# pyprob/pyprob

Measured on AMD Instinct MI355X. Metric: ic_train_traces_per_sec, higher is better.
Workload: dtype f32; 1 GPU; GaussianUnknownMean IC training, offline traces resident in HBM, LSTM hidden=512, batch=1024 per GPU; traces_in_hbm=1000000, params=1643583, global_batch=1024, parallelism=dp1, optimizer=Adam lr=1e-3*sqrt(world), launch=one Python iteration per step (ICEngine.train_step), eager launches, prewarm_steps=5670, minibatches_resident=976, minibatch_walk=step i trains minibatch (i * 1) mod 976 of the resident dataset

## Files before the change

### include/pyprob_amd.h

```cpp
#ifndef PYPROB_AMD_H
#define PYPROB_AMD_H

#include <stddef.h>
#include <stdint.h>

#ifdef __cplusplus
extern "C" {
#endif

#define PP_ABI_VERSION 15
#define PP_MAX_OBS 8
#define PP_MAX_LSTM_DEPTH 4
#define PP_MAX_OBS_DEPTH 4

#define PP_EINVAL   (-1)
#define PP_ENOSPACE (-2)
#define PP_ENODEV   (-3)
#define PP_EHIP     (-4)

#define PP_HEAD_NORMAL_MIXTURE       0
#define PP_HEAD_TRUNCNORMAL_MIXTURE  1
#define PP_HEAD_CATEGORICAL          2
#define PP_HEAD_BERNOULLI            4
#define PP_HEAD_POISSON_TN_MIXTURE   3

int         pp_abi_version(void);
const char* pp_last_error(void);
int         pp_device_count(void);

typedef struct pp_addr {
    int32_t kind;
    int32_t n_out;
    int32_t hid;
    int32_t smp_in;
    int32_t dtype_id;
    int32_t _pad;
    int64_t addr_emb;
    int64_t dtype_emb;
    int64_t smp_w;
    int64_t smp_b;
    int64_t w1, b1;
    int64_t w2, b2;
} pp_addr;

typedef struct pp_net {
    int32_t n_obs;
    int32_t obs_in[PP_MAX_OBS];
    int32_t obs_hid[PP_MAX_OBS];
    int32_t obs_out[PP_MAX_OBS];
    int64_t obs_w0[PP_MAX_OBS], obs_b0[PP_MAX_OBS], obs_w1[PP_MAX_OBS], obs_b1[PP_MAX_OBS];
    int32_t e_obs;
    int32_t smp_dim, addr_dim, dtype_dim;
    int64_t fin_w0, fin_b0, fin_w1, fin_b1;
    int32_t lstm_in;
    int32_t lstm_dim;
    int64_t w_ih, w_hh, b_ih, b_hh;
    int32_t n_addr;
    int32_t n_dtype;
    const pp_addr* addrs;
    const int64_t* addr_table;
    int64_t n_params;
    int32_t lstm_depth;
    int32_t _pad2;
    int64_t lstm_w_ih[PP_MAX_LSTM_DEPTH], lstm_w_hh[PP_MAX_LSTM_DEPTH], lstm_b_ih[PP_MAX_LSTM_DEPTH], lstm_b_hh[PP_MAX_LSTM_DEPTH];
    int32_t obs_depth[PP_MAX_OBS];
    int64_t obs_w[PP_MAX_OBS][PP_MAX_OBS_DEPTH], obs_b[PP_MAX_OBS][PP_MAX_OBS_DEPTH];
    int32_t obs_kind[PP_MAX_OBS];
    int32_t obs_shape[PP_MAX_OBS][3];
    int32_t obs_feat[PP_MAX_OBS];
    int32_t _pad3;
    int64_t obs_conv_w[PP_MAX_OBS][5], obs_conv_b[PP_MAX_OBS][5];
} pp_net;

#define PP_OBS_FEEDFORWARD 0
#define PP_OBS_CNN2D5C     1
#define PP_PROF_CNN_FWD 32
#define PP_PROF_CNN_BWD 48

size_t pp_cnn2d5c_workspace_bytes(const pp_net* net, int32_t o, int32_t n_images);
int pp_cnn2d5c_forward(const pp_net* net, int32_t o, const float* params, const float* x, int32_t n_images,
                       float* features_out, void* workspace, size_t workspace_bytes, void* stream);
int pp_cnn2d5c_backward(const pp_net* net, int32_t o, const float* params, const float* d_features, int32_t n_images,
                        float* grads, void* workspace, size_t workspace_bytes, int32_t flags, void* stream);

#define PP_ADDR_TABLE_COLS 8
#define PP_AT_KIND 0
#define PP_AT_SMP_IN 1
#define PP_AT_ADDR_EMB 2
#define PP_AT_DTYPE_EMB 3
#define PP_AT_SMP_W 4
#define PP_AT_SMP_B 5
#define PP_AT_N_OUT 6
#define PP_AT_RESERVED 7

typedef struct pp_batch {
    int32_t n_traces;
    int32_t n_rows;
    int32_t t_max;
    int32_t obs_width;
    const int32_t* n_active;
    const int32_t* row_off;
    const int32_t* grp_off;
    const float*   obs;
    const float*   value;
    const float*   prior;
    const int32_t* addr;
    const int32_t* prev_row;
    const int32_t* grp_rows;
    const int32_t* trace;
    const int32_t* row_off_dev;
    const int32_t* nxt_off;
    const int32_t* nxt_rows;
} pp_batch;

typedef struct pp_pack_info {
    int64_t n_traces, n_rows, t_max, device_words;
    int64_t obs, value, prior, addr, prev_row, grp_rows, trace, row_off_dev, nxt_rows;
    int64_t n_active, row_off, grp_off, nxt_off;
    int64_t order;
    int64_t src_row;
} pp_pack_info;

int64_t pp_pack_words(int32_t n_traces, int64_t n_rows, int32_t t_max, int32_t obs_width, int32_t n_addr);

int pp_pack_ragged(const int32_t* trace_len, const int32_t* addr_ids, const float* values, const float* prior,
                   int32_t prior_width, const float* obs, int32_t n_traces, int32_t obs_width, int32_t n_addr,
                   void* out, int64_t out_words, pp_pack_info* info);

typedef struct pp_shard_columns {
    const int32_t* trace_len;
    const int64_t* row_off;
    const float*   obs;
    const float*   value;
    const float*   prior;
    const int32_t* addr;
    const int32_t* addr_remap;
} pp_shard_columns;

int pp_pack_indexed(const pp_shard_columns* shards, int32_t n_shards, const int64_t* first, const int64_t* ids,
                    int32_t n_ids, int32_t obs_width, int32_t n_addr, void* out, int64_t out_words, pp_pack_info* info);


size_t pp_ic_workspace_bytes(const pp_net* net, int32_t n_traces, int32_t n_rows);

#define PP_LOSS_BACKWARD   1
#define PP_LOSS_ZERO_GRADS 2
#define PP_LOSS_KEEP_LP    4

int pp_ic_loss(const pp_net* net, const pp_batch* batch, const float* params , float* grads ,
               void* workspace , size_t workspace_bytes, float* loss_out ,
               int32_t* status_out , float* lp_out , int32_t flags, void* stream);

#define PP_ADAM_ZERO_GRADS 1
#define PP_ADAM_SCRATCH 1056
#define PP_ADAM_SEEN 1027
int pp_adam_step(float* params, float* grads, float* exp_avg, float* exp_avg_sq, int64_t n_params,
                 const int32_t* chunk_tensor, const float* active, int32_t* tensor_step, int32_t* scratch,
                 int32_t n_tensors, float lr, float beta1, float beta2, float eps, float weight_decay, float grad_scale,
                 int32_t flags, const int32_t* skip, void* stream);

int pp_sgd_step(float* params, float* grads, float* momentum_buf, int64_t n_params, const int32_t* chunk_tensor,
                const float* active, int32_t n_tensors, float lr, float momentum, int32_t nesterov, float weight_decay,
                float grad_scale, int32_t flags, const int32_t* skip, void* stream);

#define PP_LARC_SCRATCH_FLOATS(n_params, n_tensors) (2 * ((n_params) / 1024) + (n_tensors))
int pp_larc_scale(const float* params, float* grads, int64_t n_params, const int32_t* chunk_tensor, const float* active,
                  int32_t n_tensors, float lr, float weight_decay, float grad_scale, float trust_coefficient, float eps,
                  float epsilon, int32_t clip, float* scratch, const int32_t* skip, void* stream);

typedef struct pp_train_buffers {
    float* params; float* grads; float* exp_avg; float* exp_avg_sq;
    const int32_t* chunk_tensor; int32_t* tensor_step; int32_t* adam_scratch;
    void* workspace; size_t workspace_bytes;
    void* staging; void* device_batch; int64_t slot_words;
    float* loss_ring; int32_t* status_ring;
    int32_t n_tensors; int32_t n_slots;
    int32_t dp_world; int32_t dp_n_skip;
    int64_t dp_skip_off[4], dp_skip_cnt[4];
} pp_train_buffers;

typedef struct pp_tensor_roles {
    const int32_t* off;
    const int32_t* addr;
    const int32_t* role;
} pp_tensor_roles;

int64_t pp_train_slot_words(int32_t n_traces, int64_t n_rows, int32_t t_max, int32_t obs_width, int32_t n_addr,
                            int32_t n_tensors);

int pp_train_sync(void);
int pp_train_resident(const pp_net* net, const pp_train_buffers* tb, const pp_batch* const* batches,
                      const float* const* active, int32_t n_steps, const float* lr, float beta1, float beta2, float eps,
                      float weight_decay, int32_t grads_clean, void* stream);

int pp_train_steps(const pp_net* net, const pp_train_buffers* buffers, const pp_tensor_roles* roles,
                   const pp_shard_columns* shards, int32_t n_shards, const int64_t* first, int32_t obs_width,
                   const int64_t* ids, const int64_t* step_off, int32_t n_steps, const float* lr ,
                   float beta1, float beta2, float eps, float weight_decay, int32_t grads_clean,
                   int64_t* addr_iterations, void* stream);


size_t pp_is_workspace_bytes(const pp_net* net, int32_t n);

int pp_is_init(const pp_net* net, const float* params, const float* obs, float* e_out, void* workspace,
               size_t workspace_bytes, void* stream);

int pp_is_step(const pp_net* net, const float* params, int32_t addr_id, int32_t prev_addr_id, int32_t n,
               const float* e_obs_vec, const float* prev_value, const float* prior, int32_t prior_stride,
               float* h, float* c, int32_t state_rows, const float* value_in, float* value_out, float* logq_out,
               uint64_t seed, uint64_t offset, void* workspace, size_t workspace_bytes, void* stream);

int pp_is_step_rows(const pp_net* net, const float* params, int32_t addr_id, int32_t prev_addr_id, int32_t n,
                    const float* e_obs_vec, const float* prev_value, const float* prior, int32_t prior_stride,
                    float* h, float* c, int32_t state_rows, const int64_t* rows, const float* value_in, float* value_out,
                    float* logq_out, uint64_t seed, uint64_t offset, void* workspace, size_t workspace_bytes, void* stream);
int pp_is_step_fused_supported(const pp_net* net, int32_t addr_id, int32_t n);
int pp_is_statement_rows(const pp_net* net, const float* params, int32_t addr_id, int32_t prev_addr_id, int32_t n,
                         const float* e_obs_vec, const float* prev_value_full, const float* prior, int32_t prior_stride,
                         float* h, float* c, int32_t state_rows, const int64_t* rows, float* value_full, float* lw_full,
                         int32_t prior_kind, uint64_t seed, uint64_t offset, void* workspace, size_t workspace_bytes,
                         void* stream);

int pp_logweight_accumulate(int32_t kind, const float* p0, int32_t p0_stride, const float* p1, int32_t p1_stride,
                            const float* x, int32_t x_stride, float scale, float* lw , float* lp_out,
                            int32_t n, void* stream);

int pp_logweight_accumulate_rows(int32_t kind, const float* p0, int32_t p0_stride, const float* p1, int32_t p1_stride,
                                 const float* x, int32_t x_stride, float scale, float* lw ,
                                 const int64_t* rows, int32_t m, void* stream);

int pp_copy_rows(const float* src, int32_t src_stride, float* dst , const int64_t* rows, int32_t m, void* stream);

#define PP_PARTITION_SCRATCH(m) (((m) + 1023) / 1024 + 1)
int pp_partition_rows(const uint8_t* cond, const int64_t* rows, int32_t m, int64_t* rows_true, int64_t* rows_false,
                      int32_t* counts, int32_t* scratch, void* stream);
int pp_partition_rows_polled(const uint8_t* cond, const int64_t* rows, int32_t m, int64_t* rows_true, int64_t* rows_false,
                             int32_t* counts , int32_t seq, int32_t* scratch, void* stream);

typedef struct pp_lw_term {
    int32_t kind, p0_stride, p1_stride, x_stride;
    const float *p0, *p1, *x;
    float scale;
} pp_lw_term;
int pp_logweight_terms(const pp_lw_term* terms, int32_t count, float* lw , int32_t n, int32_t overwrite,
                       void* stream);

int pp_is_step_net(const pp_net* net, const float* params, int32_t addr_id, int32_t prev_addr_id, int32_t n,
                   const float* e_obs_vec, const float* prev_value, float* h, float* c, int32_t state_rows, void* workspace,
                   size_t workspace_bytes, void* stream);
int pp_is_first_statement_supported(const pp_net* net, int32_t addr_id);
int pp_is_first_statement(const pp_net* net, const float* params, const float* obs, int32_t addr_id, float* e_out, float* h, float* c,
                          void* workspace, size_t workspace_bytes, void* stream);
int pp_is_fused(const pp_net* net, int32_t addr_id, int32_t n, const float* prior , const pp_lw_term* terms,
                const int32_t* term_flags, int32_t n_terms, float* value , float* lw , int32_t overwrite,
                uint64_t seed, uint64_t offset, double* stats_out , double* stats_scratch, void* workspace,
                size_t workspace_bytes, void* stream);

#define PP_IS_GROUP_STATS_BYTES(m) ((size_t)((m) > 256 ? (m) : 256) * 48)
#define PP_GROUPS_PRIOR_PER_PARTICLE 2
size_t pp_is_batch_workspace_bytes(const pp_net* net, int32_t n_groups);
int pp_is_batch_first(const pp_net* net, const float* params, const float* obs , int32_t addr_id, int32_t n_groups,
                      float* y_out , int64_t ldy, float* h_out, float* c_out , void* workspace,
                      size_t workspace_bytes, void* stream);
int pp_is_fused_groups(const pp_net* net, int32_t addr_id, int32_t n_groups, int32_t n_per, const float* y , int64_t ldy,
                       const float* prior , const pp_lw_term* terms, const int32_t* term_flags, int32_t n_terms,
                       float* value , float* lw , int32_t overwrite, uint64_t seed, uint64_t offset,
                       double* stats_out , void* workspace, size_t workspace_bytes, void* stream);

int pp_is_batch_bias(const pp_net* net, const float* params, int32_t addr_id, int32_t prev_addr_id, int32_t n_groups,
                     int32_t ws_groups, int32_t first_group, const float* h_prev ,
                     float* bias_out , void* workspace, size_t workspace_bytes, void* stream);
int pp_is_statement_groups(const pp_net* net, const float* params, int32_t addr_id, int32_t prev_addr_id, int32_t n_groups,
                           int32_t n_per, const float* bias , const float* c0 ,
                           const float* prev_value , const float* prior, int32_t prior_stride, float* h, float* c,
                           float* value , float* lw , int32_t prior_kind, uint64_t seed, uint64_t offset,
                           float* y_out , int64_t ldy, void* workspace, size_t workspace_bytes,
                           void* stream);

int pp_prior_draw(int32_t kind, const float* p0, int32_t p0_stride, const float* p1, int32_t p1_stride, int32_t n, uint64_t seed,
                  uint64_t offset, uint32_t stream_id, float* out , void* stream);

int pp_obs_draw(int32_t kind, const float* p0, int64_t p0_row_stride, int32_t p0_elem_stride, const float* p1, int64_t p1_row_stride,
                int32_t p1_elem_stride, int32_t n, int32_t k, uint64_t seed, uint64_t offset, uint32_t stream_id,
                float* out , void* stream);

int pp_axpy(float scale, const float* term, float* lw, int32_t n, void* stream);

#define PP_IS_STATS_SCRATCH 6144
int pp_is_stats(const float* lw, const float* x, int32_t n, double* out, double* scratch, void* stream);

#define PP_DIST_MAX_KIND 13
#define PP_DIST_MAX_TERMS 8
#define PP_DIST_MAX_ROUNDS 64
typedef struct pp_dist {
    int32_t kind;
    int32_t p_stride[4];
    const float* p[4];
} pp_dist;
typedef struct pp_dist_term {
    pp_dist d;
    const float* x; int32_t x_stride;
    float scale;
} pp_dist_term;

int pp_dist_logweight(const pp_dist_term* terms, int32_t count, float* lw , float* lp_out, const int64_t* rows,
                      int32_t m, int32_t n, void* stream);

int pp_dist_draw(const pp_dist* d, const int64_t* rows, int32_t m, int32_t n, uint64_t seed, uint64_t offset, uint32_t stream_id,
                 float* out , void* stream);

#define PP_MIX_MAX_COMPONENTS 16
typedef struct pp_mixture {
    int32_t count;
    int32_t probs_stride;
    const float* probs;
    pp_dist comp[PP_MIX_MAX_COMPONENTS];
} pp_mixture;

int pp_mix_logweight(const pp_mixture* mix, const float* x, int32_t x_stride, float scale, float* lw , float* lp_out,
                     const int64_t* rows, int32_t m, int32_t n, void* stream);

int pp_mix_draw(const pp_mixture* mix, const int64_t* rows, int32_t m, int32_t n, uint64_t seed, uint64_t offset,
                uint32_t stream_id, float* out , void* stream);

typedef struct pp_obs_operand { const float* p; int64_t row_stride; int32_t elem_stride; int32_t _pad; } pp_obs_operand;
int pp_obs_logweight(int32_t kind, const pp_obs_operand params[4], pp_obs_operand x, int32_t k, float scale, float* lw ,
                     float* lp_out, const int64_t* rows, int32_t m, int32_t n, void* stream);

typedef struct pp_gemm_args {
    const float* A; int64_t lda; const int32_t* a_idx;
    const float* B; int64_t ldb; const int32_t* b_idx;
    float*       C; int64_t ldc; const int32_t* c_idx;
    int32_t M, N, K;
    int32_t a_kmajor, b_kmajor;
    const float* bias;
    const float* bias2;
    const float* mask; int64_t ldmask;
    int32_t relu;
    int32_t accumulate;
    float*       colsum;
    int32_t split_k;
    int32_t _pad;
} pp_gemm_args;

int pp_gemm_f32(const pp_gemm_args* args, void* stream);
int pp_gemm_f32_grouped(const pp_gemm_args* args, int32_t count, void* stream);

int pp_colsum_f32(const float* X, int64_t ldx, const int32_t* row_idx, int32_t n_rows, int32_t n_cols,
                  float* out, float* out2, void* stream);

int pp_lstm_input_gather(const pp_net* net, const float* params, const float* E, const int32_t* trace_of_row,
                         const float* value, const int32_t* addr, const int32_t* prev_row, int32_t n_rows,
                         float* X, int64_t ldx, void* stream);

int pp_lstm_cell_fwd(float* G, const float* c_prev, float* c, float* h, int32_t n, int32_t H, void* stream);
int pp_lstm_cell_bwd(float* G, const float* c_prev, const float* c, const float* dh, float* dc_carry,
                     int32_t n, int32_t n_next, int32_t H, void* stream);

int pp_head_logprob(int32_t kind, const float* y, int64_t ldy, const int32_t* rows, const float* value,
                    const float* prior, int32_t n, int32_t n_out, float grad_scale, float* lp_out, float* dy,
                    float* loss_acc, int32_t* nonfinite, void* stream);

int pp_debug_wgrad_plan(const pp_gemm_args* products, const int32_t* zero_blocks, int32_t count, int64_t* out, int32_t cap,
                        int32_t* n_blocks);
int pp_prof_arm(int32_t which, int32_t max_samples);
int pp_prof_stride(int32_t stride);
int pp_prof_collect(float* ms_out, int32_t cap, int32_t* n_out, double* flops_out);

int pp_dp_unique_id(const char* rccl_path, void* id_out );
int pp_dp_init(const char* rccl_path, const void* unique_id , int32_t rank, int32_t world);
int pp_dp_world(void);
int pp_dp_destroy(void);
int pp_dp_allreduce(float* base , const int64_t* off , const int64_t* cnt , int32_t n, void* stream);
int pp_dp_reduce_grads(float* grads_full, int64_t n_params, int32_t n_tensors, const float* presence, const int32_t* status,
                       const int64_t* skip_off , const int64_t* skip_cnt , int32_t n_skip, float* loss_out,
                       int32_t* status_out, void* stream);

int pp_dp_overlap(const int64_t* off , const int64_t* cnt , int32_t n);
int pp_dp_overlap_stats(int32_t arm, float* us_out);

int pp_debug_timeline(long long* buf );
int pp_debug_wgtrace(long long* buf, int32_t cap, int32_t mode);
int pp_debug_clock_probe(int32_t iters, long long* out , float* sink , void* stream);

#ifdef __cplusplus
}
#endif
#endif
```

### pyprob_amd/csrc/wgrad_t1.hip

```cpp
#include "wgrad_t1.hpp"

#include <stdlib.h>

#include <algorithm>

namespace pp {

extern long long* g_wgtrace;
extern int g_wgtrace_cap, g_wgtrace_mode;

namespace {

typedef float f32x16 __attribute__((ext_vector_type(16)));

constexpr int WG_RING = 8;

struct Pair {
    float a0, a1, b0, b1;
};

template <bool GATHER>
__device__ __forceinline__ void wgrad_kloop(f32x16 (&acc)[2][2], const float* __restrict__ A, const float* __restrict__ B,
                                            const int32_t* __restrict__ bidx, const int lda, const int ldb, const int M, const int N,
                                            const int m0, const int n0, const int kb, const int ke, const int lane,
                                            const bool hm, const bool hn) {
    const int l31 = lane & 31, h = lane >> 5;
    const float* pa0 = A + min(m0 + l31, M - 1);
    const float* pa1 = A + min(m0 + 32 + l31, M - 1);
    const float* pb0 = B + min(n0 + l31, N - 1);
    const float* pb1 = B + min(n0 + 32 + l31, N - 1);
    int idxA = 0, idxB = 0;
    if (GATHER) idxA = bidx[min(kb + lane, ke - 1)];
    auto load = [&](int pidx, Pair& p) {
        const int k = kb + 2 * pidx + h;
        const int kc = min(k, ke - 1);
        const float keep = k < ke ? 1.0f : 0.0f;
        p.a0 = pa0[(int64_t)kc * lda] * keep;
        p.a1 = pa1[(int64_t)kc * lda] * keep;
        int kb2 = kc;
        if (GATHER) {
            if ((pidx & 31) == 0) {
                const int nb = (pidx >> 5) + 1;
                const int v = bidx[min(kb + 64 * nb + lane, ke - 1)];
                idxB = (nb & 1) ? v : idxB;
                idxA = (nb & 1) ? idxA : v;
            }
            const int v = ((pidx >> 5) & 1) ? idxB : idxA;
            const int sel = 2 * (pidx & 31);
            const int r0 = __builtin_amdgcn_readlane(v, sel), r1 = __builtin_amdgcn_readlane(v, sel + 1);
            kb2 = h ? r1 : r0;
        }
        p.b0 = pb0[(int64_t)kb2 * ldb];
        p.b1 = pb1[(int64_t)kb2 * ldb];
    };
    auto mma = [&](const Pair& p) {
        acc[0][0] = __builtin_amdgcn_mfma_f32_32x32x2f32(p.a0, p.b0, acc[0][0], 0, 0, 0);
        if (hn) acc[0][1] = __builtin_amdgcn_mfma_f32_32x32x2f32(p.a0, p.b1, acc[0][1], 0, 0, 0);
        if (hm) acc[1][0] = __builtin_amdgcn_mfma_f32_32x32x2f32(p.a1, p.b0, acc[1][0], 0, 0, 0);
        if (hm && hn) acc[1][1] = __builtin_amdgcn_mfma_f32_32x32x2f32(p.a1, p.b1, acc[1][1], 0, 0, 0);
    };
    Pair f[WG_RING];
    const int nfr = (ke - kb + 1) >> 1;
#pragma unroll
    for (int i = 0; i < WG_RING - 1; ++i) load(i, f[i]);
    int i0 = 0;
    for (; i0 + WG_RING <= nfr; i0 += WG_RING) {
#pragma unroll
        for (int j = 0; j < WG_RING; ++j) {
            load(i0 + j + WG_RING - 1, f[(j + WG_RING - 1) % WG_RING]);
            mma(f[j]);
        }
    }
    const int nrem = nfr - i0;
#pragma unroll
    for (int j = 0; j < WG_RING - 1; ++j)
        if (j < nrem) mma(f[j]);
}

__global__ __launch_bounds__(512, 4) void wgrad_t1_kernel(const WgradT1Args g, const AuxJobs aux) {
    __shared__ float lds[8192];
    const long long t_start = g.trace ? wall_clock64() : 0;
    const int aux_lo = g.aux_first ? 0 : g.n_blocks;
    const int bx = (int)blockIdx.x - (g.aux_first ? aux.n_blocks : 0);
    if ((int)blockIdx.x >= aux_lo && (int)blockIdx.x < aux_lo + aux.n_blocks) {
        int jb = (int)blockIdx.x - aux_lo + g.aux_rot;
        if (jb >= aux.n_blocks) jb -= aux.n_blocks;
        aux_job_run(aux, jb, lds);
        if (g.trace && threadIdx.x == 0) {
            long long* tr = g.trace + 8 * blockIdx.x;
            tr[0] = t_start; tr[1] = wall_clock64(); tr[2] = 100; tr[3] = 0;
        }
        return;
    }
    int pi = 0;
#pragma unroll
    for (int q = 1; q < WGRAD_T1_MAX; ++q)
        if (q < g.n_prob && bx >= g.p[q].first) pi = q;
    const float* const A = g.p[pi].A;
    const float* const B = g.p[pi].B;
    float* const C = g.p[pi].C;
    const int32_t* const bidx = g.p[pi].bidx;
    const int lda = g.p[pi].lda, ldb = g.p[pi].ldb, ldc = g.p[pi].ldc, M = g.p[pi].M, N = g.p[pi].N, nt = g.p[pi].nt;
    const int K = g.p[pi].K, ks = g.p[pi].ks;
    const int local = bx - g.p[pi].first;
    const int mtg = g.p[pi].mtg;
    int s, tm, tn;
    if (mtg > 0) {
        const int r = local & 7, u = local >> 3;
        const int tmg = u % mtg, v = u / mtg;
        tn = v % nt;
        s = v / nt;
        tm = tmg * 8 + r;
        if (tm * 64 >= M) return;
    } else {
        const int tiles = ((M + 63) >> 6) * nt;
        s = local / tiles;
        const int t = local - s * tiles;
        tm = t / nt;
        tn = t - tm * nt;
    }
    const int tid = threadIdx.x, lane = tid & 63, l31 = lane & 31, h = lane >> 5;
    const int wave = __builtin_amdgcn_readfirstlane(tid >> 6);
    const int m0 = tm * 64, n0 = tn * 64;
    const int k0 = s * ks, k1 = min(K, k0 + ks);
    const int per = ((k1 - k0 + 15) >> 4) * 2;
    const int kb = k0 + wave * per, ke = min(k1, kb + per);
    f32x16 acc[2][2];
#pragma unroll
    for (int i = 0; i < 2; ++i)
#pragma unroll
        for (int j = 0; j < 2; ++j)
#pragma unroll
            for (int r = 0; r < 16; ++r) acc[i][j][r] = 0.0f;
    const bool hm = m0 + 32 < M, hn = n0 + 32 < N;
    if (kb < ke) {
        if (bidx) wgrad_kloop<true>(acc, A, B, bidx, lda, ldb, M, N, m0, n0, kb, ke, lane, hm, hn);
        else wgrad_kloop<false>(acc, A, B, bidx, lda, ldb, M, N, m0, n0, kb, ke, lane, hm, hn);
    }
    if (g.trace && threadIdx.x == 0) g.trace[8 * blockIdx.x + 4] = wall_clock64();
    float out[2][2][2];
#pragma unroll
    for (int qi = 0; qi < 2; ++qi) {
#pragma unroll
        for (int qj = 0; qj < 2; ++qj) {
            out[qi][qj][0] = out[qi][qj][1] = 0.0f;
            if ((qi && !hm) || (qj && !hn)) continue;
            if (qi + qj > 0) __syncthreads();
            float* mine = lds + wave * 1024 + lane;
#pragma unroll
            for (int r = 0; r < 16; ++r) mine[r * 64] = acc[qi][qj][r];
            __syncthreads();
#pragma unroll
            for (int e = 0; e < 2; ++e) {
                const int r = 2 * wave + e;
                float v = 0.0f;
#pragma unroll
                for (int w = 0; w < 8; ++w) v += lds[w * 1024 + r * 64 + lane];
                out[qi][qj][e] = v;
                if (!g.aux_first) {
                    const int gm = m0 + 32 * qi + (r & 3) + 8 * (r >> 2) + 4 * h;
                    const int gn = n0 + 32 * qj + l31;
                    if (gm < M && gn < N) atomicAdd(C + (int64_t)gm * ldc + gn, v);
                }
            }
        }
    }
#pragma unroll
    for (int qi = 0; qi < 2; ++qi)
#pragma unroll
        for (int qj = 0; qj < 2; ++qj) {
            if (!g.aux_first || (qi && !hm) || (qj && !hn)) continue;
#pragma unroll
            for (int e = 0; e < 2; ++e) {
                const int r = 2 * wave + e;
                const int gm = m0 + 32 * qi + (r & 3) + 8 * (r >> 2) + 4 * h;
                const int gn = n0 + 32 * qj + l31;
                if (gm < M && gn < N) atomicAdd(C + (int64_t)gm * ldc + gn, out[qi][qj][e]);
            }
        }
    if (g.trace && threadIdx.x == 0) {
        long long* tr = g.trace + 8 * blockIdx.x;
        tr[0] = t_start; tr[1] = wall_clock64(); tr[2] = pi; tr[3] = s;
    }
}

}

bool wgrad_t1_build(const pp_gemm_args* q, const GemmHole* holes, int n, WgradT1Args& out) {
    static const int env = getenv("PP_WGRAD_T1") ? atoi(getenv("PP_WGRAD_T1")) : 1;
    static const int env_s = 0;
    static const int env_xmap = getenv("PP_WGRAD_XMAP") ? atoi(getenv("PP_WGRAD_XMAP")) : 1;
    static const bool env_wgs_set = false;
    static const int env_wgs = 240;
    if (!env || deterministic_mode() || n <= 0) return false;
    out = WgradT1Args{};
    int np = 0;
    auto add = [&](const pp_gemm_args& a, int m_lo, int m_hi, int n_lo, int n_hi, int k_lo) -> bool {
        if (m_hi <= m_lo || n_hi <= n_lo || k_lo >= a.K) return true;
        if (np >= WGRAD_T1_MAX) return false;
        WgradT1Prob& p = out.p[np++];
        p.A = a.A + (int64_t)k_lo * a.lda + m_lo;
        p.bidx = a.b_idx ? a.b_idx + k_lo : nullptr;
        p.B = a.B + (a.b_idx ? 0 : (int64_t)k_lo * a.ldb) + n_lo;
        p.C = a.C + (int64_t)m_lo * a.ldc + n_lo;
        p.lda = (int)a.lda; p.ldb = (int)a.ldb; p.ldc = (int)a.ldc;
        p.M = m_hi - m_lo; p.N = n_hi - n_lo; p.nt = cdiv(p.N, 64);
        p.K = a.K - k_lo;
        return true;
    };
    for (int i = 0; i < n; ++i) {
        const pp_gemm_args& a = q[i];
        if (!a.a_kmajor || !a.b_kmajor || a.a_idx || a.c_idx || a.bias || a.bias2 || a.mask || a.relu || a.colsum ||
            !a.accumulate || a.K <= 0 || a.M <= 0 || a.N <= 0 || a.lda >= (1 << 30) || a.ldb >= (1 << 30) || a.ldc >= (1 << 30))
            return false;
        int mc[6] = {0, (int)a.M, 0, 0, 0, 0}, nc[6] = {0, (int)a.N, 0, 0, 0, 0};
        int nm = 2, nn = 2;
        GemmBlock z[2];
        int nz = 0;
        if (holes) {
            for (int b = 0; b < 2; ++b) {
                GemmBlock h = holes[i].b[b];
                h.m0 = std::max(h.m0, 0); h.n0 = std::max(h.n0, 0);
                h.m1 = std::min(h.m1, (int)a.M); h.n1 = std::min(h.n1, (int)a.N); h.k1 = std::min(h.k1, (int)a.K);
                if (h.m1 <= h.m0 || h.n1 <= h.n0 || h.k1 <= h.k0 || h.k0 > 0) continue;
                z[nz++] = h;
                mc[nm++] = h.m0; mc[nm++] = h.m1;
                nc[nn++] = h.n0; nc[nn++] = h.n1;
            }
        }
        std::sort(mc, mc + nm);
        std::sort(nc, nc + nn);
        nm = (int)(std::unique(mc, mc + nm) - mc);
        nn = (int)(std::unique(nc, nc + nn) - nc);
        for (int jn = 0; jn + 1 < nn; ++jn) {
            int run_lo = -1, run_hi = -1, run_k = 0;
            for (int jm = 0; jm + 1 < nm; ++jm) {
                int k_lo = 0;
                for (int b = 0; b < nz; ++b)
                    if (z[b].m0 <= mc[jm] && z[b].m1 >= mc[jm + 1] && z[b].n0 <= nc[jn] && z[b].n1 >= nc[jn + 1])
                        k_lo = std::max(k_lo, z[b].k1);
                if (run_lo >= 0 && k_lo == run_k) {
                    run_hi = mc[jm + 1];
                } else {
                    if (run_lo >= 0 && !add(a, run_lo, run_hi, nc[jn], nc[jn + 1], run_k)) return false;
                    run_lo = mc[jm]; run_hi = mc[jm + 1]; run_k = k_lo;
                }
            }
            if (run_lo >= 0 && !add(a, run_lo, run_hi, nc[jn], nc[jn + 1], run_k)) return false;
        }
    }
    if (np == 0) return false;
    int64_t tile_rows = 0;
    for (int i = 0; i < np; ++i) tile_rows += (int64_t)cdiv(out.p[i].M, 64) * out.p[i].nt * out.p[i].K;
    const int64_t blocks = env_wgs_set ? env_wgs : std::min<int64_t>(1536, std::max<int64_t>(env_wgs, tile_rows / 600));
    const int target_rows = (int)std::max<int64_t>(64, cdiv(tile_rows, std::max<int64_t>(blocks, 1)));
    out.n_prob = np;
    std::stable_sort(out.p, out.p + np, [](const WgradT1Prob& x, const WgradT1Prob& y) { return x.K > y.K; });
    int first = 0;
    for (int i = 0; i < np; ++i) {
        WgradT1Prob& p = out.p[i];
        int S = env_s > 0 ? env_s : (p.K + target_rows / 2) / target_rows;
        S = std::max(1, std::min(S, std::min(16, std::max(1, p.K / 64))));
        p.S = S;
        p.ks = ((cdiv(p.K, S) + 3) / 4) * 4;
        p.first = first;
        const int mt = cdiv(p.M, 64);
        p.mtg = (env_xmap && mt >= 8) ? cdiv(mt, 8) : 0;
        first += (p.mtg ? p.mtg * 8 : mt) * p.nt * S;
    }
    out.n_blocks = first;
    return true;
}

int wgrad_t1(const WgradT1Args& a, const AuxJobs* aux, hipStream_t st) {
    static const AuxJobs none{};
    const AuxJobs& j = aux ? *aux : none;
    const int blocks = a.n_blocks + (aux ? j.n_blocks : 0);
    WgradT1Args t = a;
    t.aux_first = (aux && a.n_blocks > 512) ? 1 : 0;
    const char* const env_rot = getenv("PP_WGRAD_JOBROT");
    if (aux && blocks <= 512 && !(env_rot && atoi(env_rot) == 0)) t.aux_rot = j.cs_first[j.n_colsum];
    if (g_wgtrace && g_wgtrace_mode == 1 && blocks <= g_wgtrace_cap) t.trace = g_wgtrace;
    hipLaunchKernelGGL(wgrad_t1_kernel, dim3(blocks), dim3(512), 0, st, t, j);
    PP_LAUNCH_CHECK("wgrad_t1");
    return 0;
}

}

extern "C" int pp_debug_wgrad_plan(const pp_gemm_args* q, const int32_t* zero_blocks, int32_t count, int64_t* out, int32_t cap,
                                   int32_t* n_blocks) {
    std::vector<pp::GemmHole> holes((size_t)std::max(count, 0));
    for (int i = 0; i < count && zero_blocks; ++i)
        for (int b = 0; b < 2; ++b) {
            const int32_t* z = zero_blocks + ((int64_t)i * 2 + b) * 6;
            holes[i].b[b] = pp::GemmBlock{z[0], z[1], z[2], z[3], z[4], z[5]};
        }
    pp::WgradT1Args a;
    if (!pp::wgrad_t1_build(q, zero_blocks ? holes.data() : nullptr, count, a)) return 0;
    if (n_blocks) *n_blocks = a.n_blocks;
    for (int i = 0; i < a.n_prob && i < cap; ++i) {
        const pp::WgradT1Prob& p = a.p[i];
        int src = -1;
        for (int k = 0; k < count; ++k)
            if (p.C >= q[k].C && p.C < q[k].C + (int64_t)q[k].M * q[k].ldc) src = k;
        int64_t* o = out + (int64_t)i * 10;
        o[0] = p.M; o[1] = p.N; o[2] = p.K; o[3] = p.S; o[4] = p.ks; o[5] = p.bidx ? 1 : 0; o[6] = p.first;
        o[7] = src >= 0 ? p.C - q[src].C : -1;
        o[8] = src >= 0 ? p.A - q[src].A : -1;
        o[9] = src >= 0 ? (p.bidx ? p.bidx - q[src].b_idx : (p.B - q[src].B)) : -1;
    }
    return a.n_prob;
}
```

### pyprob_amd/csrc/wgrad_t1.hpp

```cpp
#pragma once
#include "aux_jobs.hpp"
#include "common.hpp"

namespace pp {

constexpr int WGRAD_T1_MAX = 40;

struct WgradT1Prob {
    const float* A; const float* B; float* C;
    const int32_t* bidx;
    int lda, ldb, ldc;
    int M, N;
    int nt;
    int K, S, ks;
    int first;
    int mtg;
};

struct WgradT1Args {
    WgradT1Prob p[WGRAD_T1_MAX];
    int n_prob, n_blocks;
    int aux_first;
    int aux_rot;
    long long* trace;
};

bool wgrad_t1_build(const pp_gemm_args* q, const GemmHole* holes, int n, WgradT1Args& out);
int wgrad_t1(const WgradT1Args& a, const AuxJobs* aux, hipStream_t st);

}
```

### pyprob_amd/lib.py

```python
import ctypes as C
import os

HERE = os.path.dirname(os.path.abspath(__file__))
LIB_PATH = os.path.join(HERE, 'libpyprob_amd.so')

PP_ABI_VERSION = 15
PP_MAX_OBS = 8
PP_MAX_LSTM_DEPTH = 4
PP_MAX_OBS_DEPTH = 4
PP_MAX_MIXTURE_COMPONENTS = 16
PP_ADDR_TABLE_COLS = 8
PP_HEAD_NORMAL_MIXTURE, PP_HEAD_TRUNCNORMAL_MIXTURE, PP_HEAD_CATEGORICAL, PP_HEAD_POISSON_TN_MIXTURE = 0, 1, 2, 3
PP_HEAD_BERNOULLI = 4
PP_OBS_FEEDFORWARD, PP_OBS_CNN2D5C = 0, 1
PP_PROF_CNN_FWD, PP_PROF_CNN_BWD = 32, 48
PP_LOSS_BACKWARD, PP_LOSS_ZERO_GRADS, PP_LOSS_KEEP_LP = 1, 2, 4
PP_ADAM_ZERO_GRADS = 1
PP_ADAM_SCRATCH = 1056
PP_ADAM_SEEN = 1027


def larc_scratch_floats(n_params, n_tensors):
    return 2 * (int(n_params) // 1024) + int(n_tensors)


PP_IS_STATS_SCRATCH = 6144

i32, i64, f32p, i32p, vp = C.c_int32, C.c_int64, C.c_void_p, C.c_void_p, C.c_void_p


class pp_addr(C.Structure):
    _fields_ = [('kind', i32), ('n_out', i32), ('hid', i32), ('smp_in', i32), ('dtype_id', i32), ('_pad', i32),
                ('addr_emb', i64), ('dtype_emb', i64), ('smp_w', i64), ('smp_b', i64),
                ('w1', i64), ('b1', i64), ('w2', i64), ('b2', i64)]


class pp_net(C.Structure):
    _fields_ = [('n_obs', i32),
                ('obs_in', i32 * PP_MAX_OBS), ('obs_hid', i32 * PP_MAX_OBS), ('obs_out', i32 * PP_MAX_OBS),
                ('obs_w0', i64 * PP_MAX_OBS), ('obs_b0', i64 * PP_MAX_OBS), ('obs_w1', i64 * PP_MAX_OBS),
                ('obs_b1', i64 * PP_MAX_OBS),
                ('e_obs', i32), ('smp_dim', i32), ('addr_dim', i32), ('dtype_dim', i32),
                ('fin_w0', i64), ('fin_b0', i64), ('fin_w1', i64), ('fin_b1', i64),
                ('lstm_in', i32), ('lstm_dim', i32),
                ('w_ih', i64), ('w_hh', i64), ('b_ih', i64), ('b_hh', i64),
                ('n_addr', i32), ('n_dtype', i32),
                ('addrs', C.POINTER(pp_addr)), ('addr_table', vp), ('n_params', i64),
                ('lstm_depth', i32), ('_pad2', i32),
                ('lstm_w_ih', i64 * PP_MAX_LSTM_DEPTH), ('lstm_w_hh', i64 * PP_MAX_LSTM_DEPTH),
                ('lstm_b_ih', i64 * PP_MAX_LSTM_DEPTH), ('lstm_b_hh', i64 * PP_MAX_LSTM_DEPTH),
                ('obs_depth', i32 * PP_MAX_OBS),
                ('obs_w', (i64 * PP_MAX_OBS_DEPTH) * PP_MAX_OBS), ('obs_b', (i64 * PP_MAX_OBS_DEPTH) * PP_MAX_OBS),
                ('obs_kind', i32 * PP_MAX_OBS), ('obs_shape', (i32 * 3) * PP_MAX_OBS), ('obs_feat', i32 * PP_MAX_OBS),
                ('_pad3', i32),
                ('obs_conv_w', (i64 * 5) * PP_MAX_OBS), ('obs_conv_b', (i64 * 5) * PP_MAX_OBS)]


class pp_batch(C.Structure):
    _fields_ = [('n_traces', i32), ('n_rows', i32), ('t_max', i32), ('obs_width', i32),
                ('n_active', C.POINTER(i32)), ('row_off', C.POINTER(i32)), ('grp_off', C.POINTER(i32)),
                ('obs', vp), ('value', vp), ('prior', vp), ('addr', vp), ('prev_row', vp), ('grp_rows', vp),
                ('trace', vp), ('row_off_dev', vp), ('nxt_off', C.POINTER(i32)), ('nxt_rows', vp)]


class pp_lw_term(C.Structure):
    _fields_ = [('kind', i32), ('p0_stride', i32), ('p1_stride', i32), ('x_stride', i32),
                ('p0', vp), ('p1', vp), ('x', vp), ('scale', C.c_float)]


PP_DIST_MAX_TERMS = 8
PP_DIST_MAX_ROUNDS = 64


class pp_dist(C.Structure):
    _fields_ = [('kind', i32), ('p_stride', i32 * 4), ('p', vp * 4)]


class pp_dist_term(C.Structure):
    _fields_ = [('d', pp_dist), ('x', vp), ('x_stride', i32), ('scale', C.c_float)]


PP_MIX_MAX_COMPONENTS = 16


class pp_mixture(C.Structure):
    _fields_ = [('count', i32), ('probs_stride', i32), ('probs', vp), ('comp', pp_dist * PP_MIX_MAX_COMPONENTS)]


class pp_obs_operand(C.Structure):
    _fields_ = [('p', vp), ('row_stride', i64), ('elem_stride', i32), ('_pad', i32)]


class pp_gemm_args(C.Structure):
    _fields_ = [('A', vp), ('lda', i64), ('a_idx', vp),
                ('B', vp), ('ldb', i64), ('b_idx', vp),
                ('C', vp), ('ldc', i64), ('c_idx', vp),
                ('M', i32), ('N', i32), ('K', i32), ('a_kmajor', i32), ('b_kmajor', i32),
                ('bias', vp), ('bias2', vp), ('mask', vp), ('ldmask', i64), ('relu', i32), ('accumulate', i32),
                ('colsum', vp), ('split_k', i32), ('_pad', i32)]


class pp_pack_info(C.Structure):
    _fields_ = [(n, i64) for n in ('n_traces', 'n_rows', 't_max', 'device_words', 'obs', 'value', 'prior', 'addr', 'prev_row',
                                   'grp_rows', 'trace', 'row_off_dev', 'nxt_rows', 'n_active', 'row_off', 'grp_off',
                                   'nxt_off', 'order', 'src_row')]


class pp_shard_columns(C.Structure):
    _fields_ = [(n, vp) for n in ('trace_len', 'row_off', 'obs', 'value', 'prior', 'addr', 'addr_remap')]


class pp_train_buffers(C.Structure):
    _fields_ = [('params', vp), ('grads', vp), ('exp_avg', vp), ('exp_avg_sq', vp),
                ('chunk_tensor', vp), ('tensor_step', vp), ('adam_scratch', vp),
                ('workspace', vp), ('workspace_bytes', C.c_size_t),
                ('staging', vp), ('device_batch', vp), ('slot_words', i64),
                ('loss_ring', vp), ('status_ring', vp), ('n_tensors', i32), ('n_slots', i32),
                ('dp_world', i32), ('dp_n_skip', i32), ('dp_skip_off', i64 * 4), ('dp_skip_cnt', i64 * 4)]


class pp_tensor_roles(C.Structure):
    _fields_ = [('off', vp), ('addr', vp), ('role', vp)]


PROTOTYPES = {
    'pp_train_slot_words': (i64, [i32, i64, i32, i32, i32, i32]),
    'pp_train_sync': (C.c_int, []),
    'pp_train_resident': (C.c_int, [C.POINTER(pp_net), C.POINTER(pp_train_buffers), vp, vp, i32, vp, C.c_float, C.c_float,
                                    C.c_float, C.c_float, i32, vp]),
    'pp_train_steps': (C.c_int, [C.POINTER(pp_net), C.POINTER(pp_train_buffers), C.POINTER(pp_tensor_roles), vp, i32, vp, i32,
                                 vp, vp, i32, vp, C.c_float, C.c_float, C.c_float, C.c_float, i32, vp, vp]),
    'pp_pack_indexed': (C.c_int, [vp, i32, vp, vp, i32, i32, i32, vp, i64, vp]),
    'pp_pack_words': (i64, [i32, i64, i32, i32, i32]),
    'pp_pack_ragged': (C.c_int, [vp, vp, vp, vp, i32, vp, i32, i32, i32, vp, i64, vp]),
    'pp_cnn2d5c_workspace_bytes': (C.c_size_t, [C.POINTER(pp_net), i32, i32]),
    'pp_cnn2d5c_forward': (C.c_int, [C.POINTER(pp_net), i32, vp, vp, i32, vp, vp, C.c_size_t, vp]),
    'pp_cnn2d5c_backward': (C.c_int, [C.POINTER(pp_net), i32, vp, vp, i32, vp, vp, C.c_size_t, i32, vp]),
    'pp_abi_version': (C.c_int, []),
    'pp_last_error': (C.c_char_p, []),
    'pp_device_count': (C.c_int, []),
    'pp_ic_workspace_bytes': (C.c_size_t, [C.POINTER(pp_net), i32, i32]),
    'pp_ic_loss': (C.c_int, [C.POINTER(pp_net), C.POINTER(pp_batch), vp, vp, vp, C.c_size_t, vp, vp, vp, i32, vp]),
    'pp_adam_step': (C.c_int, [vp, vp, vp, vp, i64, vp, vp, vp, vp, i32, C.c_float, C.c_float, C.c_float, C.c_float,
                               C.c_float, C.c_float, i32, vp, vp]),
    'pp_sgd_step': (C.c_int, [vp, vp, vp, i64, vp, vp, i32, C.c_float, C.c_float, i32, C.c_float, C.c_float, i32, vp, vp]),
    'pp_larc_scale': (C.c_int, [vp, vp, i64, vp, vp, i32, C.c_float, C.c_float, C.c_float, C.c_float, C.c_float, C.c_float,
                                i32, vp, vp, vp]),
    'pp_is_workspace_bytes': (C.c_size_t, [C.POINTER(pp_net), i32]),
    'pp_is_init': (C.c_int, [C.POINTER(pp_net), vp, vp, vp, vp, C.c_size_t, vp]),
    'pp_is_step': (C.c_int, [C.POINTER(pp_net), vp, i32, i32, i32, vp, vp, vp, i32, vp, vp, i32, vp, vp, vp, C.c_uint64,
                             C.c_uint64, vp, C.c_size_t, vp]),
    'pp_is_step_rows': (C.c_int, [C.POINTER(pp_net), vp, i32, i32, i32, vp, vp, vp, i32, vp, vp, i32, vp, vp, vp, vp, C.c_uint64,
                                  C.c_uint64, vp, C.c_size_t, vp]),
    'pp_is_step_fused_supported': (C.c_int, [C.POINTER(pp_net), i32, i32]),
    'pp_is_statement_rows': (C.c_int, [C.POINTER(pp_net), vp, i32, i32, i32, vp, vp, vp, i32, vp, vp, i32, vp, vp, vp, i32,
                                       C.c_uint64, C.c_uint64, vp, C.c_size_t, vp]),
    'pp_prior_draw': (C.c_int, [i32, vp, i32, vp, i32, i32, C.c_uint64, C.c_uint64, C.c_uint32, vp, vp]),
    'pp_obs_draw': (C.c_int, [i32, vp, C.c_int64, i32, vp, C.c_int64, i32, i32, i32, C.c_uint64, C.c_uint64, C.c_uint32, vp, vp]),
    'pp_is_first_statement_supported': (C.c_int, [C.POINTER(pp_net), i32]),
    'pp_is_first_statement': (C.c_int, [C.POINTER(pp_net), vp, vp, i32, vp, vp, vp, vp, C.c_size_t, vp]),
    'pp_is_step_net': (C.c_int, [C.POINTER(pp_net), vp, i32, i32, i32, vp, vp, vp, vp, i32, vp, C.c_size_t, vp]),
    'pp_is_fused': (C.c_int, [C.POINTER(pp_net), i32, i32, vp, C.POINTER(pp_lw_term), C.POINTER(C.c_int32), i32, vp, vp, i32,
                              C.c_uint64, C.c_uint64, vp, vp, vp, C.c_size_t, vp]),
    'pp_is_batch_workspace_bytes': (C.c_size_t, [C.POINTER(pp_net), i32]),
    'pp_is_batch_first': (C.c_int, [C.POINTER(pp_net), vp, vp, i32, i32, vp, i64, vp, vp, vp, C.c_size_t, vp]),
    'pp_is_fused_groups': (C.c_int, [C.POINTER(pp_net), i32, i32, i32, vp, i64, vp, C.POINTER(pp_lw_term), C.POINTER(C.c_int32), i32,
                                     vp, vp, i32, C.c_uint64, C.c_uint64, vp, vp, C.c_size_t, vp]),
    'pp_is_batch_bias': (C.c_int, [C.POINTER(pp_net), vp, i32, i32, i32, i32, i32, vp, vp, vp, C.c_size_t, vp]),
    'pp_is_statement_groups': (C.c_int, [C.POINTER(pp_net), vp, i32, i32, i32, i32, vp, vp, vp, vp, i32, vp, vp, vp, vp, i32,
                                         C.c_uint64, C.c_uint64, vp, i64, vp, C.c_size_t, vp]),
    'pp_logweight_accumulate': (C.c_int, [i32, vp, i32, vp, i32, vp, i32, C.c_float, vp, vp, i32, vp]),
    'pp_logweight_accumulate_rows': (C.c_int, [i32, vp, i32, vp, i32, vp, i32, C.c_float, vp, vp, i32, vp]),
    'pp_copy_rows': (C.c_int, [vp, i32, vp, vp, i32, vp]),
    'pp_partition_rows': (C.c_int, [vp, vp, i32, vp, vp, vp, vp, vp]),
    'pp_partition_rows_polled': (C.c_int, [vp, vp, i32, vp, vp, vp, i32, vp, vp]),
    'pp_logweight_terms': (C.c_int, [C.POINTER(pp_lw_term), i32, vp, i32, i32, vp]),
    'pp_axpy': (C.c_int, [C.c_float, vp, vp, i32, vp]),
    'pp_is_stats': (C.c_int, [vp, vp, i32, vp, vp, vp]),
    'pp_dist_logweight': (C.c_int, [C.POINTER(pp_dist_term), i32, vp, vp, vp, i32, i32, vp]),
    'pp_dist_draw': (C.c_int, [C.POINTER(pp_dist), vp, i32, i32, C.c_uint64, C.c_uint64, C.c_uint32, vp, vp]),
    'pp_mix_logweight': (C.c_int, [C.POINTER(pp_mixture), vp, i32, C.c_float, vp, vp, vp, i32, i32, vp]),
    'pp_obs_logweight': (C.c_int, [i32, C.POINTER(pp_obs_operand), pp_obs_operand, i32, C.c_float, vp, vp, vp, i32, i32, vp]),
    'pp_mix_draw': (C.c_int, [C.POINTER(pp_mixture), vp, i32, i32, C.c_uint64, C.c_uint64, C.c_uint32, vp, vp]),
    'pp_gemm_f32': (C.c_int, [C.POINTER(pp_gemm_args), vp]),
    'pp_gemm_f32_grouped': (C.c_int, [C.POINTER(pp_gemm_args), i32, vp]),
    'pp_colsum_f32': (C.c_int, [vp, i64, vp, i32, i32, vp, vp, vp]),
    'pp_lstm_input_gather': (C.c_int, [C.POINTER(pp_net), vp, vp, vp, vp, vp, vp, i32, vp, i64, vp]),
    'pp_lstm_cell_fwd': (C.c_int, [vp, vp, vp, vp, i32, i32, vp]),
    'pp_lstm_cell_bwd': (C.c_int, [vp, vp, vp, vp, vp, i32, i32, i32, vp]),
    'pp_head_logprob': (C.c_int, [i32, vp, i64, vp, vp, vp, i32, i32, C.c_float, vp, vp, vp, vp, vp]),
    'pp_debug_clock_probe': (C.c_int, [i32, vp, vp, vp]),
    'pp_dp_unique_id': (C.c_int, [C.c_char_p, vp]),
    'pp_dp_init': (C.c_int, [C.c_char_p, vp, i32, i32]),
    'pp_dp_world': (C.c_int, []),
    'pp_dp_destroy': (C.c_int, []),
    'pp_dp_allreduce': (C.c_int, [vp, vp, vp, i32, vp]),
    'pp_dp_reduce_grads': (C.c_int, [vp, i64, i32, vp, vp, vp, vp, i32, vp, vp, vp]),
    'pp_dp_overlap': (C.c_int, [vp, vp, i32]),
    'pp_dp_overlap_stats': (C.c_int, [i32, vp]),
    'pp_debug_timeline': (C.c_int, [vp]),
    'pp_debug_wgtrace': (C.c_int, [vp, C.c_int32, C.c_int32]),
    'pp_debug_wgrad_plan': (C.c_int, [vp, vp, i32, vp, i32, vp]),
    'pp_prof_arm': (C.c_int, [i32, i32]),
    'pp_prof_stride': (C.c_int, [i32]),
    'pp_prof_collect': (C.c_int, [vp, i32, vp, vp]),
}

_lib = None


class HipLibraryError(RuntimeError):
    pass


def load():
    global _lib
    if _lib is not None:
        return _lib
    import torch
    if not os.path.exists(LIB_PATH):
        raise HipLibraryError('%s not found: build it with `python -m pyprob_amd.build` (hipcc, gfx950). '
                              'pyprob_amd has no CPU fallback.' % LIB_PATH)
    try:
        lib = C.CDLL(LIB_PATH)
    except OSError as e:
        raise HipLibraryError('cannot load %s: %s' % (LIB_PATH, e))
    for name, (res, args) in PROTOTYPES.items():
        fn = getattr(lib, name)
        fn.restype = res
        fn.argtypes = args
    if lib.pp_abi_version() != PP_ABI_VERSION:
        raise HipLibraryError('ABI version mismatch: library %d, binding %d' % (lib.pp_abi_version(), PP_ABI_VERSION))
    _lib = lib
    return lib


def check(rc, what=''):
    if rc != 0:
        msg = load().pp_last_error()
        raise RuntimeError('libpyprob_amd %s failed (rc=%d): %s' % (what, rc, msg.decode() if msg else ''))


def ptr(t):
    return None if t is None else t.data_ptr()


_raw_stream = None


def stream_ptr(device_index=None):
    global _raw_stream
    import torch
    if _raw_stream is None:
        _raw_stream = getattr(torch._C, '_cuda_getCurrentRawStream', False)
    if _raw_stream:
        return _raw_stream(torch.cuda.current_device() if device_index is None else device_index)
    return torch.cuda.current_stream().cuda_stream
```

Before: 16.62 million traces/s.

## Add wide vectorized 16x16x4 MFMA path for weight-gradient tiles

Adds a second weight-gradient tile kernel that, when A and B are 16-byte aligned and the leading dimensions allow it, loads up to four contiguous floats per lane and accumulates with 16x16x4 f32 MFMA into a 4x4 block of accumulators. Gathered B rows are fetched by shuffling index values across lanes with readlane. Cross-wave partial sums are reduced through a larger, swizzled LDS buffer before the atomic adds. This aims to cut load instruction count and raise MFMA density per byte loaded. In exchange it doubles static LDS per block, which may lower occupancy, and adds register pressure and many template variants. A debug entry point for running the planner is also added.

```diff
diff --git a/include/pyprob_amd.h b/include/pyprob_amd.h
--- a/include/pyprob_amd.h
+++ b/include/pyprob_amd.h
@@ -363,6 +363,8 @@
 
 int pp_debug_wgrad_plan(const pp_gemm_args* products, const int32_t* zero_blocks, int32_t count, int64_t* out, int32_t cap,
                         int32_t* n_blocks);
+int pp_debug_wgrad_run(const pp_gemm_args* products, const int32_t* zero_blocks, int32_t count, int32_t launch, void* stream,
+                       int32_t* wide_out, int32_t cap);
 int pp_prof_arm(int32_t which, int32_t max_samples);
 int pp_prof_stride(int32_t stride);
 int pp_prof_collect(float* ms_out, int32_t cap, int32_t* n_out, double* flops_out);
diff --git a/pyprob_amd/csrc/wgrad_t1.hip b/pyprob_amd/csrc/wgrad_t1.hip
--- a/pyprob_amd/csrc/wgrad_t1.hip
+++ b/pyprob_amd/csrc/wgrad_t1.hip
@@ -77,8 +77,172 @@
         if (j < nrem) mma(f[j]);
 }
 
+typedef float f32x4 __attribute__((ext_vector_type(4)));
+typedef float f32x2 __attribute__((ext_vector_type(2)));
+
+constexpr int WG_RINGW = 5;
+constexpr int WG_RINGW_GATHER = 4;
+
+template <int MB, int NB>
+struct Quad {
+    float a[MB], b[NB];
+};
+
+template <int W>
+__device__ __forceinline__ void load_vec(float (&d)[W], const float* __restrict__ p) {
+    if constexpr (W == 4) {
+        const f32x4 v = *reinterpret_cast<const f32x4*>(p);
+        d[0] = v[0]; d[1] = v[1]; d[2] = v[2]; d[3] = v[3];
+    } else if constexpr (W == 2) {
+        const f32x2 v = *reinterpret_cast<const f32x2*>(p);
+        d[0] = v[0]; d[1] = v[1];
+    } else {
+        d[0] = *p;
+    }
+}
+
+template <bool GATHER, int MB, int NB>
+__device__ __forceinline__ void wgrad_kloop_wide(f32x4 (&acc)[4][4], const float* __restrict__ A, const float* __restrict__ B,
+                                                 const int32_t* __restrict__ bidx, const int lda, const int ldb, const int M,
+                                                 const int N, const int m0, const int n0, const int kb, const int ke,
+                                                 const int lane) {
+    const int c = lane & 15, q = lane >> 4;
+    const float* pa = A + (MB == 1 ? min(m0 + c, M - 1) : m0 + MB * c);
+    const float* pb = B + (NB == 1 ? min(n0 + c, N - 1) : n0 + NB * c);
+    int cur = 0, nxt = 0;
+    if (GATHER) {
+        cur = bidx[min(kb + lane, ke - 1)];
+        nxt = bidx[min(kb + 64 + lane, ke - 1)];
+        asm volatile("" : "+v"(nxt));
+    }
+    const int q_odd = -(q & 1), q_hi = -(q >> 1);
+    auto load = [&](int pidx, Quad<MB, NB>& p, bool site) {
+        const int k = kb + 4 * pidx + q;
+        const int kc = min(k, ke - 1);
+        load_vec<MB>(p.a, pa + (int64_t)kc * lda);
+        int kb2 = kc;
+        if (GATHER) {
+            if (site) {
+                cur = (pidx & 15) == 0 ? nxt : cur;
+                nxt = bidx[min(kb + 64 * ((pidx >> 4) + 1) + lane, ke - 1)];
+            }
+            const int v = cur;
+            const int sel = 4 * (pidx & 15);
+            const int r0 = __builtin_amdgcn_readlane(v, sel), r1 = __builtin_amdgcn_readlane(v, sel + 1);
+            const int r2 = __builtin_amdgcn_readlane(v, sel + 2), r3 = __builtin_amdgcn_readlane(v, sel + 3);
+            const int t0 = r0 ^ ((r0 ^ r1) & q_odd), t1 = r2 ^ ((r2 ^ r3) & q_odd);
+            kb2 = t0 ^ ((t0 ^ t1) & q_hi);
+        }
+        load_vec<NB>(p.b, pb + (int64_t)kb2 * ldb);
+    };
+    auto mma = [&](int pidx, const Quad<MB, NB>& p) {
+        const float keep = kb + 4 * pidx + q < ke ? 1.0f : 0.0f;
+#pragma unroll
+        for (int i = 0; i < MB; ++i) {
+            const float a = p.a[i] * keep;
+#pragma unroll
+            for (int j = 0; j < NB; ++j) acc[i][j] = __builtin_amdgcn_mfma_f32_16x16x4f32(a, p.b[j], acc[i][j], 0, 0, 0);
+        }
+    };
+    constexpr int RING = GATHER ? WG_RINGW_GATHER : WG_RINGW;
+    static_assert(WG_RINGW_GATHER == 4, "the index blocks' reload sits at every fourth quad-row");
+    Quad<MB, NB> f[RING];
+    const int nfr = (ke - kb + 3) >> 2;
+#pragma unroll
+    for (int i = 0; i < RING - 1; ++i) load(i, f[i], false);
+    int i0 = 0;
+    for (; i0 + RING <= nfr; i0 += RING) {
+#pragma unroll
+        for (int j = 0; j < RING; ++j) {
+            load(i0 + j + RING - 1, f[(j + RING - 1) % RING], ((j + RING - 1) & 3) == 0);
+            __builtin_amdgcn_sched_barrier(0);
+            mma(i0 + j, f[j]);
+            __builtin_amdgcn_sched_barrier(0);
+        }
+    }
+    const int nrem = nfr - i0;
+#pragma unroll
+    for (int j = 0; j < RING - 1; ++j)
+        if (j < nrem) mma(i0 + j, f[j]);
+}
+
+template <int MB, int NB>
+__device__ __forceinline__ void wgrad_kloop_wide_any(f32x4 (&acc)[4][4], const float* A, const float* B, const int32_t* bidx,
+                                                     const int lda, const int ldb, const int M, const int N, const int m0,
+                                                     const int n0, const int kb, const int ke, const int lane) {
+    if (bidx) wgrad_kloop_wide<true, MB, NB>(acc, A, B, bidx, lda, ldb, M, N, m0, n0, kb, ke, lane);
+    else wgrad_kloop_wide<false, MB, NB>(acc, A, B, bidx, lda, ldb, M, N, m0, n0, kb, ke, lane);
+}
+
+__device__ __forceinline__ void wgrad_tile_wide(const WgradT1Args& g, const WgradT1Prob& p, const int m0, const int n0, const int k0,
+                                                const int k1, float* lds) {
+    const float* const A = p.A;
+    const float* const B = p.B;
+    float* const C = p.C;
+    const int32_t* const bidx = p.bidx;
+    const int lda = p.lda, ldb = p.ldb, ldc = p.ldc, M = p.M, N = p.N;
+    const int tid = threadIdx.x, lane = tid & 63, c = lane & 15, q = lane >> 4;
+    const int wave = __builtin_amdgcn_readfirstlane(tid >> 6);
+    const int per = ((k1 - k0 + 31) >> 5) * 4;
+    const int kb = k0 + wave * per, ke = min(k1, kb + per);
+    const int mb = M - m0 > 32 ? 4 : M - m0 > 16 ? 2 : 1, nb = N - n0 > 32 ? 4 : N - n0 > 16 ? 2 : 1;
+    f32x4 acc[4][4];
+#pragma unroll
+    for (int i = 0; i < 4; ++i)
+#pragma unroll
+        for (int j = 0; j < 4; ++j) acc[i][j] = f32x4{0.0f, 0.0f, 0.0f, 0.0f};
+    if (kb < ke) {
+#define PP_WIDE_CASE(MB, NB) \
+    case MB * 8 + NB: wgrad_kloop_wide_any<MB, NB>(acc, A, B, bidx, lda, ldb, M, N, m0, n0, kb, ke, lane); break;
+        switch (mb * 8 + nb) {
+            PP_WIDE_CASE(4, 4) PP_WIDE_CASE(4, 2) PP_WIDE_CASE(4, 1)
+            PP_WIDE_CASE(2, 4) PP_WIDE_CASE(2, 2) PP_WIDE_CASE(2, 1)
+            PP_WIDE_CASE(1, 4) PP_WIDE_CASE(1, 2) PP_WIDE_CASE(1, 1)
+        }
+#undef PP_WIDE_CASE
+    }
+    if (g.trace && threadIdx.x == 0) g.trace[8 * blockIdx.x + 4] = wall_clock64();
+    const int si = wave >> 2, sq = wave & 3;
+    const int oc = lane >> 2, oj = lane & 3;
+    f32x4 out[2];
+    auto add_out = [&](int h, const f32x4& v) {
+        const int i = 2 * h + si, gn = n0 + nb * oc + oj;
+        if (i >= mb || oj >= nb || gn >= N) return;
+#pragma unroll
+        for (int r = 0; r < 4; ++r) {
+            const int gm = m0 + mb * (4 * sq + r) + i;
+            if (gm < M) atomicAdd(C + (int64_t)gm * ldc + gn, v[r]);
+        }
+    };
+    const int wr = wave * 2048 + q * 256 + 16 * c, swz = (c >> 1) & 3;
+    const int rd = wave * 256 + 4 * ((lane & ~3) | (oj ^ ((lane >> 3) & 3)));
+#pragma unroll
+    for (int h = 0; h < 2; ++h) {
+        if (2 * h >= mb) break;
+        if (h) __syncthreads();
+#pragma unroll
+        for (int il = 0; il < 2; ++il)
+            if (2 * h + il < mb) {
+#pragma unroll
+                for (int j = 0; j < 4; ++j) *reinterpret_cast<f32x4*>(lds + wr + il * 1024 + 4 * (j ^ swz)) = acc[2 * h + il][j];
+            }
+        __syncthreads();
+        f32x4 v = f32x4{0.0f, 0.0f, 0.0f, 0.0f};
+        if (2 * h + si < mb) {
+#pragma unroll
+            for (int w = 0; w < 8; ++w) v += *reinterpret_cast<const f32x4*>(lds + w * 2048 + rd);
+        }
+        out[h] = v;
+        if (!g.aux_first) add_out(h, v);
+    }
+    if (g.aux_first) {
+        add_out(0, out[0]);
+        if (mb > 2) add_out(1, out[1]);
+    }
+}
+
 __global__ __launch_bounds__(512, 4) void wgrad_t1_kernel(const WgradT1Args g, const AuxJobs aux) {
-    __shared__ float lds[8192];
+    __shared__ __attribute__((aligned(16))) float lds[16384];
     const long long t_start = g.trace ? wall_clock64() : 0;
     const int aux_lo = g.aux_first ? 0 : g.n_blocks;
     const int bx = (int)blockIdx.x - (g.aux_first ? aux.n_blocks : 0);
@@ -119,6 +283,14 @@
         tm = t / nt;
         tn = t - tm * nt;
     }
+    if (g.p[pi].wide) {
+        wgrad_tile_wide(g, g.p[pi], tm * 64, tn * 64, s * ks, min(K, s * ks + ks), lds);
+        if (g.trace && threadIdx.x == 0) {
+            long long* tr = g.trace + 8 * blockIdx.x;
+            tr[0] = t_start; tr[1] = wall_clock64(); tr[2] = pi; tr[3] = s;
+        }
+        return;
+    }
     const int tid = threadIdx.x, lane = tid & 63, l31 = lane & 31, h = lane >> 5;
     const int wave = __builtin_amdgcn_readfirstlane(tid >> 6);
     const int m0 = tm * 64, n0 = tn * 64;
@@ -193,8 +365,16 @@
     static const bool env_wgs_set = false;
     static const int env_wgs = 240;
     if (!env || deterministic_mode() || n <= 0) return false;
+    const char* const env_wide = getenv("PP_WGRAD_WIDE");
+    const bool wide_on = !(env_wide && atoi(env_wide) == 0);
     out = WgradT1Args{};
     int np = 0;
+    auto vec_ok = [](const float* ptr, int64_t ld, int lo, int ext) {
+        if (((uintptr_t)ptr & 15) || (ld & 3)) return false;
+        const int t0 = (ext - 1) / 64 * 64, rem = ext - t0;
+        const int w = rem > 32 ? 4 : rem > 16 ? 2 : 1;
+        return w == 1 || (int64_t)lo + t0 + 16 * w <= ld;
+    };
     auto add = [&](const pp_gemm_args& a, int m_lo, int m_hi, int n_lo, int n_hi, int k_lo) -> bool {
         if (m_hi <= m_lo || n_hi <= n_lo || k_lo >= a.K) return true;
         if (np >= WGRAD_T1_MAX) return false;
@@ -206,6 +386,7 @@
         p.lda = (int)a.lda; p.ldb = (int)a.ldb; p.ldc = (int)a.ldc;
         p.M = m_hi - m_lo; p.N = n_hi - n_lo; p.nt = cdiv(p.N, 64);
         p.K = a.K - k_lo;
+        p.wide = (wide_on && vec_ok(p.A, a.lda, m_lo, p.M) && vec_ok(p.B, a.ldb, n_lo, p.N)) ? 1 : 0;
         return true;
     };
     for (int i = 0; i < n; ++i) {
@@ -312,3 +493,18 @@
     }
     return a.n_prob;
 }
+
+extern "C" int pp_debug_wgrad_run(const pp_gemm_args* q, const int32_t* zero_blocks, int32_t count, int32_t launch, void* stream,
+                                  int32_t* wide_out, int32_t cap) {
+    std::vector<pp::GemmHole> holes((size_t)std::max(count, 0));
+    for (int i = 0; i < count && zero_blocks; ++i)
+        for (int b = 0; b < 2; ++b) {
+            const int32_t* z = zero_blocks + ((int64_t)i * 2 + b) * 6;
+            holes[i].b[b] = pp::GemmBlock{z[0], z[1], z[2], z[3], z[4], z[5]};
+        }
+    pp::WgradT1Args a;
+    if (!pp::wgrad_t1_build(q, zero_blocks ? holes.data() : nullptr, count, a)) return 0;
+    for (int i = 0; i < a.n_prob && i < cap && wide_out; ++i) wide_out[i] = a.p[i].wide;
+    if (launch && pp::wgrad_t1(a, nullptr, (hipStream_t)stream) != 0) return 0;
+    return a.n_prob;
+}
diff --git a/pyprob_amd/csrc/wgrad_t1.hpp b/pyprob_amd/csrc/wgrad_t1.hpp
--- a/pyprob_amd/csrc/wgrad_t1.hpp
+++ b/pyprob_amd/csrc/wgrad_t1.hpp
@@ -15,6 +15,7 @@
     int K, S, ks;
     int first;
     int mtg;
+    int wide;
 };
 
 struct WgradT1Args {
diff --git a/pyprob_amd/lib.py b/pyprob_amd/lib.py
--- a/pyprob_amd/lib.py
+++ b/pyprob_amd/lib.py
@@ -201,6 +201,7 @@
     'pp_debug_timeline': (C.c_int, [vp]),
     'pp_debug_wgtrace': (C.c_int, [vp, C.c_int32, C.c_int32]),
     'pp_debug_wgrad_plan': (C.c_int, [vp, vp, i32, vp, i32, vp]),
+    'pp_debug_wgrad_run': (C.c_int, [vp, vp, i32, i32, vp, vp, i32]),
     'pp_prof_arm': (C.c_int, [i32, i32]),
     'pp_prof_stride': (C.c_int, [i32]),
     'pp_prof_collect': (C.c_int, [vp, i32, vp, vp]),
```

After: 17.05 million traces/s, median of 6. 1.03x the previous value.
